# brucefan1983/GPUMD

Measured on AMD Instinct MI355X. Metric: atom-steps/sec, NEP PbTe NVE (nep4 2 Te Pb, examples/nep_train/nep.txt), higher is better.
Workload: dtype f32

## Files before the change

gpumd_amd/csrc/capi_impl.h:

```cpp
#pragma once
#include "../../include/nepmi.h"
#include "engine_impl.h"

#include <exception>
#include <string>

struct nepmi_api;
#if defined(NEPMI_CAPI_DISPATCH)
extern "C" const nepmi_api nepmi_self_api;
#define NEPMI_SELF_API (&nepmi_self_api)
#else
#define NEPMI_SELF_API nullptr
#endif

struct nepmi_model {
  const nepmi_api* api;
  nepmi::NepModel m;
};

struct nepmi_engine {
  const nepmi_api* api;
  nepmi::EngineT<NepmiBackend>* e;
};

// ... 525 lines not shown
    return guarded([&] { eng.set_force_generic(iv != 0); });
  if (n == "tiles")
    eng.set_tile_mode(iv < 0 ? -1 : iv > 2 ? 2 : iv);
  else if (n == "win_lanes")
    eng.set_win_lanes(iv);
  else if (n == "win_max_atoms")
    eng.set_win_max_atoms(iv);
  else if (n == "scatter_guard")
    eng.set_scatter_guard_delayed(value, eng.take_guard_delay());
  else if (n == "scatter_guard_hard")
    eng.set_scatter_guard(-1.0, value);
  else if (n == "scatter_guard_delay")
    eng.set_guard_delay(iv);
  else if (n == "radial_mask")
    eng.set_radial_mask(iv != 0);
  else if (n == "radial_sync")
    eng.set_radial_sync(iv != 0);
  else if (n == "angular_fused")
    eng.set_angular_fused(iv != 0);
  else if (n == "angular_pair_trip")
    eng.set_angular_pair_trip(iv != 0);
  else if (n == "fold_seam")
    eng.set_fold_seam(iv != 0);
  else if (n == "brick_force") {
    if (iv != 0 && !eng.has_brick_force())
      return fail(NEPMI_ERR_ARG, "option 'brick_force': the per-brick force kernel is not part of this build (make BRICK=1)");
    eng.set_brick_force(iv != 0);
  }
  else if (n == "win_static")
    eng.set_win2(iv != 0);
  else if (n == "stepwise_loops")
    eng.set_stepwise_loops(iv != 0);
  else if (n == "mfma")
    eng.set_use_mfma(iv);
  else if (n == "angular_recompute")
    eng.set_angular_recompute(iv);
  else
    return fail(NEPMI_ERR_ARG, "unknown engine option '" + n + "'");
  return NEPMI_OK;
}

}
```

gpumd_amd/csrc/engine.hip:

```cpp
#include <hip/hip_runtime.h>
#include <hiprand/hiprand_kernel.h>

#include <cstring>
#include <stdexcept>
#include <string>

#include "engine_impl.h"
#include "nep_scatter.h"
#include "nep_fused.h"
#ifndef NEPMI_WITH_BRICK
#define NEPMI_WITH_BRICK 0
#endif
#if NEPMI_WITH_BRICK
#include "experimental/nep_brick.h"
#endif

namespace nepmi {

#define NEPMI_HIP_CHECK(expr)                                                                       \
  do {                                                                                              \
    hipError_t err__ = (expr);                                                                      \
    if (err__ != hipSuccess)                                                                        \
      throw std::runtime_error(std::string("HIP error: ") + hipGetErrorString(err__) + " at " +     \
                               __FILE__ + ":" + std::to_string(__LINE__) + " (" #expr ")");         \
// ... 292 lines not shown
  const unsigned per_xcd = gridDim.x >> 3;
  const int64_t wg = (int64_t)(blockIdx.x & 7u) * per_xcd + (blockIdx.x >> 3);
  const int64_t i0 = wg * 128;
  if (i0 >= n)
    return;
  const int tid = (int)threadIdx.x;
  const int64_t i = i0 + (tid >> 1);
  const bool live = i < n;
  const int64_t k = body.b.tperm[live ? i : i0];
  const int t1 = body.b.posq[k].type;
  const int64_t ilast = i0 + 127 < n ? i0 + 127 : n - 1;
  const int t_lo = body.b.posq[body.b.tperm[i0]].type, t_hi = body.b.posq[body.b.tperm[ilast]].type;
  for (int tb = t_lo; tb <= t_hi; tb += kFusedWindowTypes) {
    const int nt = body.m.T - tb < kFusedWindowTypes ? body.m.T - tb : kFusedWindowTypes;
    __syncthreads();
    body.stage_window(nepmi_lds_window, tb, nt, tid, 256);
    __syncthreads();
    if (live && t1 >= tb && t1 < tb + nt)
      body.run_window(k, tid & 1, (lds_cfloat_ptr)nepmi_lds_window, tb);
  }
}
#endif

template <int BLOCK, class Body>
__global__ void __launch_bounds__(BLOCK) __attribute__((amdgpu_waves_per_eu(Body::kMinWavesPerEuPairs)))
nepmi_kernel_lds_pairs_sorted(const Body body, const int64_t n, const int* frozen)
{
  extern __shared__ __attribute__((aligned(16))) float nepmi_lds_pairs_s[];
  __shared__ int hist[64];
  __shared__ unsigned short perm[BLOCK / 2];
  if (frozen && *frozen != 0)
    return;
  const int tid = (int)threadIdx.x;
  body.lds_stage(nepmi_lds_pairs_s, tid, BLOCK);
  if (tid < 64)
    hist[tid] = 0;
  const unsigned per_xcd = gridDim.x >> 3;
  const unsigned tile = (blockIdx.x & 7u) * per_xcd + (blockIdx.x >> 3);
  const int64_t base = (int64_t)tile * (BLOCK / 2);
  const int j = tid >> 1;
  const bool live = base + j < n;
  int key = 0;
  if (live) {
    key = body.sort_key(base + j);
    key = key > 63 ? 63 : key;
    if (tile & 1u)
      key = 63 - key;
  }
  __syncthreads();
  if (live && (tid & 1) == 0)
    atomicAdd(&hist[key], 1);
  __syncthreads();
  if (tid == 0) {
    int run = 0;
    for (int c = 63; c >= 0; --c) {
      const int h = hist[c];
      hist[c] = run;
      run += h;
    }
  }
  __syncthreads();
  if (live && (tid & 1) == 0)
    perm[atomicAdd(&hist[key], 1)] = (unsigned short)j;
  __syncthreads();
  if (live)
    body.template run_parts<2>(base + perm[j], tid & 1, (lds_cfloat_ptr)nepmi_lds_pairs_s);
}

template <class Body>
__global__ void __launch_bounds__(256) nepmi_fused_image(const Body body, float* img)
{
  body.lds_stage(img, (int)threadIdx.x, 256);
}

template <int BLOCK, int P, class Body>
__global__ void __launch_bounds__(BLOCK) nepmi_kernel_lds_parts(const Body body, const int64_t n, const int* frozen)
{
  extern __shared__ __attribute__((aligned(16))) float nepmi_lds_parts[];
  if (frozen && *frozen != 0)
    return;
  const unsigned per_xcd = gridDim.x >> 3;
  const unsigned tile = (blockIdx.x & 7u) * per_xcd + (blockIdx.x >> 3);
  const int64_t i = ((int64_t)tile * BLOCK + threadIdx.x) / P;
  if (i < n)
    body.template run_parts<P>(i, (int)(threadIdx.x % P), (lds_cfloat_ptr)nepmi_lds_parts);
}

template <int BLOCK>
__device__ __forceinline__ int block_exclusive_scan(int v, int* total);
// ... 991 lines not shown
    hipLaunchKernelGGL((nepmi_kernel_lds<BLOCK, Body>), dim3((unsigned)grid), dim3(BLOCK), lds_bytes, stream, body, n, frozen);
    NEPMI_HIP_CHECK(hipGetLastError());
    if (t)
      timer_stop(timing->slot[slot]);
  }

  template <int BLOCK, int P, class Body>
  void launch_lds_parts(int slot, int64_t n, const Body& body)
  {
    if (n <= 0)
      return;
    const int64_t grid = ((P * n + BLOCK - 1) / BLOCK + 7) / 8 * 8;
    const size_t lds_bytes = ((size_t)body.lds_floats() * sizeof(float) + 15) / 16 * 16;
    const bool t = timed(slot);
    if (t)
      timer_start(timing->slot[slot]);
    hipLaunchKernelGGL((nepmi_kernel_lds_parts<BLOCK, P, Body>), dim3((unsigned)grid), dim3(BLOCK), lds_bytes, stream, body, n,
                       frozen);
    NEPMI_HIP_CHECK(hipGetLastError());
    if (t)
      timer_stop(timing->slot[slot]);
  }

  template <int BLOCK, class Body, bool SORTED = false>
  void launch_lds_pairs(int slot, int64_t n, const Body& body)
  {
    if (n <= 0)
      return;
    const int64_t grid = ((2 * n + BLOCK - 1) / BLOCK + 7) / 8 * 8;
    const size_t lds_bytes = ((size_t)body.lds_floats() * sizeof(float) + 15) / 16 * 16;
    void (*kern)(const Body, const int64_t, const int*) = nullptr;
    if constexpr (SORTED)
      kern = &nepmi_kernel_lds_pairs_sorted<BLOCK, Body>;
    else
      kern = &nepmi_kernel_lds_pairs<BLOCK, Body>;
    if (lds_bytes > 60 * 1024)
      NEPMI_HIP_CHECK(hipFuncSetAttribute(reinterpret_cast<const void*>(kern), hipFuncAttributeMaxDynamicSharedMemorySize, (int)lds_bytes));
    const bool t = timed(slot);
    if (t)
      timer_start(timing->slot[slot]);
    hipLaunchKernelGGL(kern, dim3((unsigned)grid), dim3(BLOCK), lds_bytes, stream, body, n, frozen);
    NEPMI_HIP_CHECK(hipGetLastError());
    if (t)
      timer_stop(timing->slot[slot]);
  }

  template <class S>
  size_t fused_image_floats(const ModelD& md) const
  {
    return (size_t)fused_lds_layout<S>(md).total;
  }
  template <class S>
  void launch_angular_fused(int slot, int64_t n, const ModelD& md, const Bufs& b, int export_qfp, float* img, bool build, bool pair_trip)
  {
    AngularFusedBody<S> body{md, b, export_qfp, nullptr};
    if (build) {
      hipLaunchKernelGGL((nepmi_fused_image<AngularFusedBody<S>>), dim3(1), dim3(256), 0, stream, body, img);
      NEPMI_HIP_CHECK(hipGetLastError());
    }
    body.img = img;
#ifndef NEPMI_AFU_BLOCK
#define NEPMI_AFU_BLOCK 256
#endif
#ifndef NEPMI_AFU_SORT
#define NEPMI_AFU_SORT 0
#endif
    if constexpr (FusedShape<S>::NLOC <= kFusedTripMaxChannels) {
      if (pair_trip) {
        launch_lds_pairs<NEPMI_AFU_BLOCK, AngularFusedBody<S, 1>, NEPMI_AFU_SORT != 0>(slot, n, AngularFusedBody<S, 1>{md, b, export_qfp, img});
        return;
      }
    }
    launch_lds_pairs<NEPMI_AFU_BLOCK, AngularFusedBody<S>, NEPMI_AFU_SORT != 0>(slot, n, body);
  }

  template <class S>
  size_t fused_window_lds_bytes(const ModelD& md) const
  {
    return (size_t)fused_lds_layout<S>(md, kFusedWindowTypes).total * sizeof(float);
  }
  static constexpr bool kHasFusedWindow = NEPMI_WITH_FUSED_WINDOW != 0;
  template <class S>
  void launch_angular_fused_window(int slot, int64_t n, const ModelD& md, const Bufs& b, int export_qfp, float* img, bool build)
  {
#if NEPMI_WITH_FUSED_WINDOW
    if (n <= 0)
      return;
    AngularFusedBody<S> body{md, b, export_qfp, nullptr};
    if (build) {
      hipLaunchKernelGGL((nepmi_fused_image<AngularFusedBody<S>>), dim3(1), dim3(256), 0, stream, body, img);
      NEPMI_HIP_CHECK(hipGetLastError());
    }
    body.img = img;
    body.tw = kFusedWindowTypes;
    const int64_t grid = ((n + 127) / 128 + 7) / 8 * 8;
    const size_t lds_bytes = (fused_window_lds_bytes<S>(md) + 15) / 16 * 16;
// ... 438 lines not shown
```

gpumd_amd/csrc/engine_impl.h:

```cpp
#pragma once
#include "nep_bodies.h"
#include "nep_md.h"
#include "nep_model.h"
#include "nep_window.h"
#include "nep_highl.h"
#include "tersoff_bodies.h"

#include <cmath>
#include <cstdio>
#include <cstring>
#include <string>
#include <random>
#include <vector>

#ifndef NEPMI_TERSOFF_SEAM
#define NEPMI_TERSOFF_SEAM 1
#endif
#ifndef NEPMI_WIN2_DEFAULT
#define NEPMI_WIN2_DEFAULT 1
#endif

#define NEPMI_UNPAREN(...) __VA_ARGS__
#if defined(NEPMI_JIT_CORE)
#define NEPMI_SHAPE_DISPATCH(FN, GENERIC, ARGS)                                   \
// ... 995 lines not shown
    const double ras = m.rc_angular_max + kSkin;
    b_.MN_ang = (int)(1.5 * m.MN_angular * ras * ras * ras / (m.rc_angular_max * m.rc_angular_max * m.rc_angular_max)) + 4;
    if (b_.MN_ang > b_.MN_skin)
      b_.MN_ang = b_.MN_skin;
    if (b_.MN_ang > 65000)
      throw EngineError{-3, "angular Verlet list capacity above 65000 slots is not supported"};
    b_.rc_skin_sq = (float)(rcs * rcs);
    b_.rc_askin_sq = (float)(ras * ras);
    b_.cid = dalloc<int>(N);
    b_.kcell = dalloc<int>(N);
    b_.perm = dalloc<int>(N);
    b_.posq = dalloc<PosQ>(N);
    b_.x0s = dalloc<double>(3 * N);
    b_.nn_skin = dalloc<int>(N);
    b_.nl_skin = dalloc<int>((size_t)b_.MN_skin * N);
    b_.code_skin = dalloc<unsigned short>((size_t)b_.MN_skin * N);
    b_.nn_ang = dalloc<int>(N);
    b_.nl_ang = dalloc<int>((size_t)b_.MN_ang * N);
    b_.code_ang = dalloc<unsigned short>((size_t)b_.MN_ang * N);
    b_.rev_ang = dalloc<unsigned short>((size_t)b_.MN_ang * N);
    b_.nn_rad = dalloc<int>(N);
    b_.nn_angstep = dalloc<int>(N);
    b_.nn_angtrue = dalloc<int>(N);
    if (m.kind == 0) {
      b_.rstash = dalloc<F4>((size_t)(b_.MN_ang + b_.MN_skin) * N);
      b_.acomp = dalloc<F4>((size_t)b_.MN_arows * N);
      b_.amap = dalloc<unsigned short>((size_t)b_.MN_ang * N);
      b_.f12 = dalloc<F4>((size_t)b_.MN_arows * N);
      b_.q = dalloc<float>((size_t)m.dim * N);
      b_.fp = dalloc<float>((size_t)m.dim * N);
      b_.sbuf = dalloc<float>((size_t)(m.n_max_angular + 1) * kNumHarm * N);
      b_.shi = m.L_max > 4 ? dalloc<float>((size_t)(m.n_max_angular + 1) * kHighSums * N) : nullptr;
      b_.KRP = ((m.basis_size_radial + 1) + 3) / 4 * 4;
      b_.atab = dalloc<float>((size_t)N * m.num_types * b_.KRP);
      const AnnMfmaShape as = ann_mfma_shape(m.num_types, m.dim, m.num_neurons, b_.KRP);
      b_.ann_img = as.ok ? dalloc<float>(as.img_floats * m.num_types) : nullptr;
      be_.ann_prepare(md_, b_);
      b_.pe_i = dalloc<float>(N);
      b_.MN_rad = m.MN_radial;
      b_.ccode = dalloc<unsigned short>((size_t)b_.MN_rad * N);
      b_.nn_t0 = dalloc<int>(N);
      b_.prec = dalloc<WinRec>(N);
      b_.aidx = dalloc<unsigned short>((size_t)b_.MN_acomp * N);
      b_.amask = dalloc<unsigned>(4 * (size_t)N);
      b_.MN_wchunks = (b_.MN_ang + 3) / 4 + 2 * ((b_.MN_skin + 3) / 4) + 4;
      b_.wcode = dalloc<unsigned short>((size_t)b_.MN_wchunks * 4 * N);
// ... 411 lines not shown
    if constexpr (B::kHasFusedWindow && B::kHasFusedAngular && S::fixed && S::TS == 0) {
      const size_t need = be_.template fused_image_floats<S>(md_);
      if (!fused_img_ || fused_img_floats_ < need) {
        dfree(fused_img_);
        fused_img_ = dalloc<float>(need);
        fused_img_floats_ = need;
        fused_img_stale_ = true;
      }
      be_.template launch_angular_fused_window<S>(kSlotAngular, N_, md_, b_, export_qfp, fused_img_, fused_img_stale_);
      fused_img_stale_ = false;
    }
  }
  template <class S>
  void launch_angular_fused(int export_qfp = 0)
  {
    if constexpr (B::kHasFusedAngular && S::fixed) {
      const size_t need = be_.template fused_image_floats<S>(md_);
      if (!fused_img_ || fused_img_floats_ < need) {
        dfree(fused_img_);
        fused_img_ = dalloc<float>(need);
        fused_img_floats_ = need;
        fused_img_stale_ = true;
      }
      be_.template launch_angular_fused<S>(kSlotAngular, N_, md_, b_, export_qfp, fused_img_, fused_img_stale_, ang_pair_trip_);
      fused_img_stale_ = false;
    }
  }

  template <class S>
  bool brick_force_wanted(const WinStage& ws2) const
  {
    if constexpr (!(B::kHasBrickForce && S::fixed && S::TS == 2)) {
      return false;
    } else {
      if (!brick_force_ || !ang_fused_active() || b_.level || b_.use_rmask || b_.use_csync || !scatter_wanted<S>(ws2))
        return false;
      return be_.template brick_lds_bytes<S>(md_, win_.wmax) <= B::kMaxLdsBytes;
    }
  }
  template <class S>
  void launch_brick_force(const WinStage& ws2, const int* frozen)
  {
    if constexpr (B::kHasBrickForce && S::fixed && S::TS == 2) {
      if (fused_img_stale_ || !fused_img_) {
        launch_angular_fused<S>(0);
      }
      be_.template launch_brick_force<S>(kSlotAngular, kSlotForce, num_bricks_, N_, ws2, md_, halo_, fmap_, fold_rows_, step_outputs_,
// ... 122 lines not shown
    fused_img_stale_ = true;
  }
  double temperature() const { return temperature_; }
  bool temperature_model() const { return model_.temperature_model; }
  int recompute_s() const
  {
    return recompute_mode_ < 0 ? (model_.MN_angular <= 16 ? 1 : 0) : (recompute_mode_ ? 1 : 0);
  }
  void adopt_from(const EngineT& o)
  {
    use_tiles_ = o.use_tiles_;
    tile_mode_ = o.tile_mode_;
    recompute_mode_ = o.recompute_mode_;
    win_lanes_ = o.win_lanes_;
    win_max_atoms_ = o.win_max_atoms_;
    use_win2_ = o.use_win2_;
    external_skin_ = o.external_skin_;
    force_form_ = o.force_form_;
    use_rmask_ = o.use_rmask_;
    use_csync_ = o.use_csync_;
    ang_fused_ = o.ang_fused_;
    ang_pair_trip_ = o.ang_pair_trip_;
    fold_seam_ = o.fold_seam_;
    brick_force_ = o.brick_force_;
    loop_ctx_ = o.loop_ctx_;
    scatter_disabled_ = o.scatter_disabled_;
    b_.scatter_limit = o.b_.scatter_limit;
    b_.fold_guard = o.b_.fold_guard;
    b_.scatter_hard = o.b_.scatter_hard;
    b_.fold_hard = o.b_.fold_hard;
    hard_factor_ = o.hard_factor_;
    hard_asked_ = o.hard_asked_;
    guard_delay_ = o.guard_delay_;
    guard_delayed_ = o.guard_delayed_;
    if (reverse_ghosts_ != o.reverse_ghosts_)
      set_reverse_ghosts(o.reverse_ghosts_);
    unwrapped_ = o.unwrapped_;
    nhc_fresh_ = o.nhc_fresh_;
    bdp_rng_ = o.bdp_rng_;
    bdp_iset_ = o.bdp_iset_;
    bdp_gset_ = o.bdp_gset_;
    lan_seed_ = o.lan_seed_;
    num_compute = o.num_compute;
    num_rebuild = o.num_rebuild;
    num_discarded = o.num_discarded;
    num_range_handovers = o.num_range_handovers;
// ... 335 lines not shown
  }
  bool scatter_enabled() const { return !scatter_disabled_; }
  void clear_range_hard()
  {
    int ov = 0;
    be_.d2h(&ov, b_.flags + kFlagOverflow, sizeof(int));
    if (ov & kOverflowRangeHard) {
      ov &= ~kOverflowRangeHard;
      be_.h2d(b_.flags + kFlagOverflow, &ov, sizeof(int));
    }
  }
  void disable_scatter()
  {
    if (!scatter_disabled_)
      ++num_range_handovers;
    scatter_disabled_ = true;
    be_.memset(b_.flags + kFlagRange, 0, sizeof(int));
  }
  bool last_scatter_form() const { return last_scatter_form_; }
  void set_angular_fused(bool on) { ang_fused_ = on; }
  void set_angular_pair_trip(bool on) { ang_pair_trip_ = on; }
  bool ang_pair_trip_active() const { return ang_pair_trip_ && (model_.n_max_angular + 2) / 2 <= 4; }
  void set_fold_seam(bool on) { fold_seam_ = on; }
  void set_brick_force(bool on) { brick_force_ = on; }
  static constexpr bool has_brick_force() { return B::kHasBrickForce; }
  void set_loop_context(bool on) { loop_ctx_ = on; }
  void set_step_outputs(bool on) { step_outputs_ = on; }
  bool loop_context() const { return loop_ctx_; }
  void exact_virials()
  {
    if (!virial_local_ || model_.kind != 0 || last_small_)
      return;
    be_.frozen = nullptr;
    NEPMI_SHAPE_DISPATCH(exact_virials_shape, 1, ())
  }
  bool virial_local() const { return virial_local_; }

private:
  template <class S>
  void compact_lists_shape()
  {
    const bool padded_rows = b_.use_csync != 0;
    force_kernels_shape<S>(kPhaseRadialOnly, nullptr);
    if (padded_rows)
      angular_kernels<S>();
  }
// ... 71 lines not shown
    } else {
      if (shape_ == 7 || shape_ == 8 || shape_ == 9) {
        s += shape_ == 7 ? "shape=cover(8,12,8,12,6;T)" : (shape_ == 8 ? "shape=cover(12,16,10,12,6;T)" : "shape=cover(8,12,8,12,6;2)");
        if (model_.embedded()) {
          char eb[128];
          std::snprintf(eb, sizeof eb, "<-zero_padded_model(%d,%d,%d,%d,%d)", model_.file_n_max_radial, model_.file_basis_size_radial,
                        model_.file_n_max_angular, model_.file_basis_size_angular, model_.file_num_L);
          s += eb;
        }
      } else {
        s += std::string("shape=") + shapes[shape_ >= 0 && shape_ <= 5 ? shape_ : 0];
      }
    }
    if (last_small_)
      return s + " path=small_box(all image pairs)";
    const int lanes = win_lanes();
    const bool win2 = win2_ok_ && lanes == 1;
    s += tile_ok_ ? (win2 ? " window=lds_static" : " window=lds_scanned") : " window=none(gather kernels)";
    s += " lanes_per_atom=" + std::to_string(tile_ok_ ? lanes : 1);
    if (last_brick_)
      s += " force=one_kernel_per_brick(descriptor+ann+partial_forces+lds_scatter_of_own_halves,lane_pairs)";
    else if (last_ang_fused_)
      s += last_ang_window_ ? " angular=descriptor+ann+partial_forces_in_one_kernel(lane_pairs,sums_in_registers,type_sorted,window_of_4_types)"
                            : (ang_pair_trip_active() ? " angular=descriptor+ann+partial_forces_in_one_kernel(lane_pairs,sums_in_registers,two_record_trips)"
                                              : " angular=descriptor+ann+partial_forces_in_one_kernel(lane_pairs,sums_in_registers)");
    else if (fuse_ann_active())
      s += " ann=fused_with_angular_descriptor(packed_fp32,no_mfma)";
    else if (ann_mode_ != 0 && b_.ann_img && (model_.num_types <= 4 || b_.skip_atab))
      s += model_.num_types > 4 ? " ann=mfma_f32_32x32x2(one_type_per_workgroup)" : " ann=mfma_f32_32x32x2";
    else
      s += " ann=per_atom";
    if (!last_ang_fused_) {
      s += (shape_ != 0 && model_.n_max_angular + 1 >= 7) ? " angular_force=lane_pairs" : " angular_force=one_lane";
      s += recompute_s() ? " angular_sums=recomputed" : " angular_sums=stored";
    }
    s += (last_scatter_form_ && last_mask_form_)   ? " radial_list=inside_bits_over_the_verlet_words"
         : (last_scatter_form_ && last_sync_form_) ? " radial_list=wave_synchronous_words"
                                                   : " radial_list=compacted";
    s += last_scatter_form_ ? (last_fold_seam_ ? " force_assembly=lds_scatter_of_own_halves(fixed_point)+fold_in_integrator_pass"
                                               : " force_assembly=lds_scatter_of_own_halves(fixed_point)+fold") :
         last_rows_form_ ? " force_assembly=table_rows_in_lds"
                         : (last_fpj_form_ ? " force_assembly=neighbour_half_from_fp_rows" : " force_assembly=table_rows_gathered");
    if (num_seam_vetoes_ > 0)
      s += " seam_vetoes=" + std::to_string(num_seam_vetoes_);
    if (tile_ok_)
      s += " bricks=" + std::to_string(num_bricks_) + " window_slots=" + std::to_string(win_.wmax);
    return s;
  }
// ... 32 lines not shown
      be_.end_region(kRegionForce);
      return;
    }
    NEPMI_SHAPE_DISPATCH(force_kernels_shape, 1, (phase, frozen))
  }

  NepModel model_;
  B be_;
  int64_t cap_;
  int64_t N_;
  ModelD md_{};
  Bufs b_;
  BoxD box_;
  WinLayout win_{0, 0};
  bool win2_ok_ = false, use_win2_ = NEPMI_WIN2_DEFAULT != 0;
  bool use_rows_ = true;
  bool last_rows_form_ = false, last_fpj_form_ = false, last_scatter_form_ = false;
  int force_form_ = -1;
  bool loop_ctx_ = false;
  bool virial_local_ = false;
  double hard_factor_ = 4.0;
  bool ang_fused_ = true;
  bool ang_pair_trip_ = !(std::getenv("NEPMI_ANGULAR_PAIR_TRIP") && std::atoi(std::getenv("NEPMI_ANGULAR_PAIR_TRIP")) == 0);
  bool brick_force_ = false;
  bool last_brick_ = false;
  bool brick_pending_ = false;
  float* fused_img_ = nullptr;
  size_t fused_img_floats_ = 0;
  bool fused_img_stale_ = true;
  bool last_ang_fused_ = false;
  bool use_rmask_ = false;
  bool last_mask_form_ = false;
  bool last_ang_window_ = false;
  bool last_sync_form_ = false;
  int guard_delay_ = 0;
  int guard_delay_next_ = 0;
  bool fold_seam_ = !(std::getenv("NEPMI_FOLD_SEAM") && std::atoi(std::getenv("NEPMI_FOLD_SEAM")) == 0);
  bool fold_defer_ = false;
  bool fold_deferred_ = false;
  static constexpr int kSeamBackoffSteps = 256;
  int seam_backoff_ = 0;
  int64_t num_seam_vetoes_ = 0;
  bool last_fold_seam_ = false;
  bool tersoff_defer_ = false;
  bool tersoff_deferred_ = false;
  int64_t calm_steps_ = 0;
// ... 81 lines not shown
```

gpumd_amd/csrc/nep_bodies.h:

```cpp
#pragma once
#include <type_traits>

#include "nep_dev.h"

namespace nepmi {

struct alignas(16) F4 {
  float x, y, z;
  int w;
};

struct alignas(16) U4 {
  unsigned x, y, z, w;
};

struct alignas(16) WinRec {
  int x, y, z;
  int w;
};

struct WinGeom {
  double inv_unit;
  double cell_frac[3];
  int cv[9];
// ... 48 lines not shown
  int gbx, gby, gbz;
  double rc_inv_cell;
  float rc_skin_sq;
  float rc_askin_sq;
  int* cell_count;
  int* cell_fill;
  int* cell_ghost;
  int* brick_live;
  int* brick_flag;
  int* brick_order;
  int* cid;
  int* perm;
  PosQ* posq;
  double* x0s;
  int MN_skin, MN_ang, MN_acomp;
  int MN_arows;
  int* nn_ang;   int* nl_ang;  unsigned short* rev_ang;
  int* nn_skin;  int* nl_skin;
  unsigned short* code_ang;
  unsigned short* code_skin;
  int* nn_rad;   F4* rstash;
  int* nn_angstep; F4* acomp;
  int* nn_angtrue;
  unsigned short* amap;
  F4* f12;
  float* q;
  float* fp;
  float* sbuf;
  float* shi;
  float* atab;
  int KRP;
  float* ann_img;
  float* pe_i;
  float* zbl;
  int* flags;
  const signed char* level;
  signed char* lvl;
  signed char lvl_desc = 1, lvl_force = 2;
  signed char* angf;
  int* tperm;
  int* tpos;
  int* tcount;
  int* sh_ang;
  double* fo;
  int MN_rad;
  unsigned short* ccode;
// ... 1297 lines not shown
      const float d = sqrtf(dot3f(e.x, e.x, e.y, e.y, e.z, e.z));
      const float rc = (rc1 + m.rc_r[t2]) * 0.5f;
      const float rcinv = fast_rcp(rc);
      float fc;
      cutoff_fc(rcinv, d, fc);
      float fn[S::KRM + 1];
      if (S::fixed)
        basis_fn<S::KRM>(rcinv, d, fc, fn);
      else
        basis_fn_rt(KR, rcinv, d, fc, fn);
      const float* c = m.c_rad + (size_t)(t1 * m.T + t2) * (NR + 1) * (KR + 1);
      for (int n = 0; n <= NR; ++n) {
        float g = 0.0f;
        for (int kk = 0; kk <= KR; ++kk)
          g += fn[kk] * c[n * (KR + 1) + kk];
        q[n] += g;
      }
    }
    for (int n = 0; n <= NR; ++n)
      b.q[(int64_t)n * N + b.tpos[k]] = q[n] * m.qscale[n];
  }
};

template <class S, int PARTS, class LP>
NEPMI_HD void angular_s_sums_scalar(const ModelD& m, const Bufs& b, int64_t k, int t1, LP cang, int part, float* s)
{
  constexpr int NLOC = (S::NAM + PARTS) / PARTS;
  const int64_t N = b.N;
  const int NA = S::fixed ? S::NA : m.NA;
  const int KA = S::fixed ? S::KA : m.KA;
  const float rc1 = m.rc_a[t1];
  const int cstride = cang_stride(m);
#pragma unroll
  for (int a = 0; a < NLOC * kNumHarm; ++a)
    s[a] = 0.0f;
  const int na = b.nn_angstep[k];
  const F4* __restrict__ acomp = b.acomp + k;
  F4 e_next;
  if (na > 0)
    e_next = acomp[0];
  for (int a = 0; a < na; ++a) {
    const F4 e = e_next;
    if (a + 1 < na)
      e_next = acomp[(int64_t)(a + 1) * N];
    if (e.w == kNullRecord)
      continue;
// ... 26 lines not shown
        g = fmaf(fn[kk], c[n * (KA + 1) + kk], g);
      }
#pragma unroll
      for (int h = 0; h < kNumHarm; ++h)
        s[i * kNumHarm + h] = fmaf(g, bh[h], s[i * kNumHarm + h]);
    }
  }
}

template <class S, int PARTS, class LP>
NEPMI_HD void angular_s_sums(const ModelD& m, const Bufs& b, int64_t k, int t1, LP cang, int part, float* s)
{
  if constexpr (!S::fixed) {
    angular_s_sums_scalar<S, PARTS>(m, b, k, t1, cang, part, s);
  } else {
    constexpr int NLOC = (S::NAM + PARTS) / PARTS;
    const int64_t N = b.N;
    const float rc1 = m.rc_a[t1];
    const int cstride = cang_stride(m);
    f2 s2[NLOC * kHarmPairs];
#pragma unroll
    for (int a = 0; a < NLOC * kHarmPairs; ++a)
      s2[a] = bc2(0.0f);
    const int na = b.nn_angstep[k];
    const F4* __restrict__ acomp = b.acomp + k;
    F4 e_next;
    if (na > 0)
      e_next = acomp[0];
    for (int a = 0; a < na; ++a) {
      const F4 e = e_next;
      if (a + 1 < na)
        e_next = acomp[(int64_t)(a + 1) * N];
      if (e.w == kNullRecord)
        continue;
      const int t2 = (int)((unsigned)e.w >> kIdxBits);
      const float x = e.x, y = e.y, z = e.z;
      float d, dinv;
      dist_and_inv(dot3f(x, x, y, y, z, z), d, dinv);
      const float rc = m.uniform_rc ? m.rc_a_max : (rc1 + m.rc_a[t2]) * 0.5f;
      const float rcinv = fast_rcp(rc);
      float fc;
      cutoff_fc(rcinv, d, fc);
      float fn[S::KAM + 1];
      basis_fn<S::KAM>(rcinv, d, fc, fn);
      f2 bh[kHarmPairs];
      harmonics_pairs(x * dinv, y * dinv, z * dinv, bh);
      LP c = cang + (t1 * m.T + t2) * cstride;
// ... 15 lines not shown
    const int hp[kNumHarm] = NEPMI_HARM_PAIR_INIT;
#pragma unroll
    for (int i = 0; i < NLOC; ++i)
#pragma unroll
      for (int q = 0; q < kHarmPairs; ++q) {
        s[i * kNumHarm + hp[2 * q]] = s2[i * kHarmPairs + q].x;
        s[i * kNumHarm + hp[2 * q + 1]] = s2[i * kHarmPairs + q].y;
      }
  }
}

template <class S, class LP>
NEPMI_HD void angular_s_sums_trip(const ModelD& m, const Bufs& b, int64_t k, int t1, LP cang, int part, float* s)
{
  static_assert(S::fixed, "compiled shapes only");
  constexpr int NLOC = (S::NA + 2) / 2;
  const int64_t N = b.N;
  const float rc1 = m.rc_a[t1];
  const int cstride = cang_stride(m);
  f2 s2[NLOC * kHarmPairs];
#pragma unroll
  for (int a = 0; a < NLOC * kHarmPairs; ++a)
    s2[a] = bc2(0.0f);
  const int na = b.nn_angstep[k];
  const F4* __restrict__ acomp = b.acomp + k;
  F4 e_next;
  e_next.x = e_next.y = e_next.z = 1.0f;
  e_next.w = kNullRecord;
  if (part < na)
    e_next = acomp[(int64_t)part * N];
  for (int a = 0; a < na; a += 2) {
    const F4 e = e_next;
    e_next.w = kNullRecord;
    if (a + 2 + part < na)
      e_next = acomp[(int64_t)(a + 2 + part) * N];
    const int wA = NEPMI_PAIR_EVEN(e.w), wB = NEPMI_PAIR_ODD(e.w);
    if (wA == kNullRecord && wB == kNullRecord)
      continue;
    const int t2 = e.w != kNullRecord ? (int)((unsigned)e.w >> kIdxBits) : 0;
    const float x = e.x, y = e.y, z = e.z;
    float d, dinv;
    dist_and_inv(dot3f(x, x, y, y, z, z), d, dinv);
    const float rc = m.uniform_rc ? m.rc_a_max : (rc1 + m.rc_a[t2]) * 0.5f;
    const float rcinv = fast_rcp(rc);
    float fc;
    cutoff_fc(rcinv, d, fc);
    float fn[S::KA + 1];
// ... 461 lines not shown
    const int NA = S::fixed ? S::NA : m.NA;
    const int KA = S::fixed ? S::KA : m.KA;
    const float rc1 = m.rc_a[t1];
    const int cstride = cang_stride(m);
    constexpr int NG2 = S::fixed ? NLOC * kHarmPairs : 1;
    f2 G2[NG2];
    if constexpr (S::fixed) {
      const int hp[kNumHarm] = NEPMI_HARM_PAIR_INIT;
#pragma unroll
      for (int i = 0; i < NLOC; ++i)
#pragma unroll
        for (int q = 0; q < kHarmPairs; ++q)
          G2[i * kHarmPairs + q] = mk2(G[i * kNumHarm + hp[2 * q]], G[i * kNumHarm + hp[2 * q + 1]]);
    }

    float zf[3] = {0, 0, 0}, zv[6] = {0, 0, 0, 0, 0, 0}, zpe = 0.0f;
    float pzi = 0.0f;
    int zi = 0;
    if (m.zbl_enabled) {
      zi = m.atomic_number[t1];
      pzi = powf((float)zi, 0.23f);
    }

    const int na = b.nn_angstep[k];
    const F4* __restrict__ acomp = b.acomp + k;
    F4 e_next;
    if (na > 0)
      e_next = acomp[0];
    for (int a = 0; a < na; ++a) {
      const F4 e = e_next;
      if (a + 1 < na)
        e_next = acomp[(int64_t)(a + 1) * N];
      if (e.w == kNullRecord)
        continue;
      const int t2 = (int)((unsigned)e.w >> kIdxBits);
      const float x = e.x, y = e.y, z = e.z;
      float d, dinv;
      dist_and_inv(dot3f(x, x, y, y, z, z), d, dinv);
      const float rc = m.uniform_rc ? m.rc_a_max : (rc1 + m.rc_a[t2]) * 0.5f;
      const float rcinv = fast_rcp(rc);
      float fc, fcp;
      cutoff_fc_fcp(rcinv, d, fc, fcp);
      float fn[S::KAM + 1], fnp[S::KAM + 1];
      if (S::fixed)
        basis_fn_fnp<S::KAM>(rcinv, d, fc, fcp, fn, fnp);
      else
        basis_fn_fnp_rt(KA, rcinv, d, fc, fcp, fn, fnp);
// ... 96 lines not shown
    if (m.zbl_enabled) {
      zi = m.atomic_number[t1];
      pzi = powf((float)zi, 0.23f);
    }
    auto share = [&](const f2* gg, float rx, float ry, float rz, float& w, float& vx, float& vy, float& vz) __attribute__((always_inline)) {
      f2 P2[kHarmPairs], Q2[kHarmPairs];
#pragma unroll
      for (int q = 0; q < kHarmPairs; ++q)
        P2[q] = Q2[q] = bc2(0.0f);
#pragma unroll
      for (int i = 0; i < NLOC; ++i) {
        if (part + 2 * i > S::NA)
          break;
        const f2 g2 = bc2(gg[i].x), gp2 = bc2(gg[i].y);
#pragma unroll
        for (int q = 0; q < kHarmPairs; ++q) {
          P2[q] = vfma(G2[i * kHarmPairs + q], g2, P2[q]);
          Q2[q] = vfma(G2[i * kHarmPairs + q], gp2, Q2[q]);
        }
      }
      harmonics_contract_pairs(rx, ry, rz, P2, Q2, w, vx, vy, vz);
    };

    const int na = b.nn_angstep[k];
    const F4* __restrict__ acomp = b.acomp + k;
    F4 e_next;
    e_next.x = e_next.y = e_next.z = 1.0f;
    e_next.w = kNullRecord;
    if (part < na)
      e_next = acomp[(int64_t)part * N];
    for (int a = 0; a < na; a += 2) {
      const F4 e = e_next;
      e_next.w = kNullRecord;
      if (a + 2 + part < na)
        e_next = acomp[(int64_t)(a + 2 + part) * N];
      const bool own = e.w != kNullRecord, partner = NEPMI_PAIR_XCHG(e.w) != kNullRecord;
      if (!own && !partner)
        continue;
      const int t2 = own ? (int)((unsigned)e.w >> kIdxBits) : 0;
      const float x = e.x, y = e.y, z = e.z;
      float d, dinv;
      dist_and_inv(dot3f(x, x, y, y, z, z), d, dinv);
      const float rc = m.uniform_rc ? m.rc_a_max : (rc1 + m.rc_a[t2]) * 0.5f;
      const float rcinv = fast_rcp(rc);
      float fc, fcp;
      cutoff_fc_fcp(rcinv, d, fc, fcp);
      float fn[S::KA + 1], fnp[S::KA + 1];
// ... 335 lines not shown
```

gpumd_amd/csrc/nep_fused.h:

```cpp
#pragma once
#include "nep_window.h"

namespace nepmi {

template <class S>
struct FusedShape {
  static_assert(S::fixed, "compiled shapes only");
  static constexpr int NRH = (S::NR + 2) / 2;
  static constexpr int NLOC = (S::NA + 2) / 2;
  static constexpr int DPH = (NRH + S::NL * NLOC + 3) / 4 * 4;
  NEPMI_HD static int component(int part, int i)
  {
    if (i < NRH) {
      const int n = 2 * i + part;
      return n <= S::NR ? n : -1;
    }
    const int ii = i - NRH, L = ii / NLOC, c = ii - L * NLOC, n = 2 * c + part;
    if (L >= S::NL || n > S::NA)
      return -1;
    return (S::NR + 1) + L * (S::NA + 1) + n;
  }
};

constexpr int kFusedTripMaxChannels = 4;
// ... 78 lines not shown
    for (int idx = tid; idx < m.T * per_t; idx += nth) {
      const int t = idx / per_t, r = idx - t * per_t;
      const int j = r / (2 * F::DPH), pi = r - j * (2 * F::DPH);
      const int p = pi / F::DPH, i = pi - p * F::DPH;
      const int d = F::component(p, i);
      dst[a.off_w + t * a.wstride + r] = d >= 0 ? m.w0[((size_t)t * m.nneu + j) * m.dim + d] : 0.0f;
    }
    for (int idx = tid; idx < m.T * m.nneu; idx += nth) {
      dst[a.off_b0 + idx] = m.b0[idx];
      dst[a.off_w1 + idx] = m.w1[idx];
    }
    for (int idx = tid; idx < m.T * m.T * (m.NR + 1) * (m.KR + 1); idx += nth)
      dst[a.off_c + idx] = m.c_rad[idx];
    for (int idx = tid; idx < 2 * F::DPH; idx += nth) {
      const int d = F::component(idx / F::DPH, idx % F::DPH);
      dst[a.off_qs + idx] = d >= 0 ? m.qscale[d] : 0.0f;
    }
  }

  NEPMI_HD int sort_key(int64_t k) const
  {
    if (b.lvl[k] < b.lvl_desc)
      return 0;
    return (b.use_csync && b.nn_angtrue) ? b.nn_angtrue[k] : b.nn_angstep[k];
  }
  template <int PARTS, class LP>
  NEPMI_HD void run_parts(int64_t k, int part, LP lds) const
  {
    static_assert(PARTS == 2, "lane pairs");
    run_window(k, part, lds, 0);
  }
  template <class LP>
  NEPMI_HD void run_window(int64_t k, int part, LP lds, int tb) const
  {
    constexpr int NLOC = F::NLOC, DPH = F::DPH;
    if (b.lvl[k] < b.lvl_desc)
      return;
    const int t1 = b.posq[k].type;
    LP cang = lds - tb * m.T * cang_stride(m);
    float s[NLOC * kNumHarm], Fp[DPH], e;
    descriptor_and_ann(k, part, lds, cang, t1, t1 - tb, s, Fp, e);
    if (part == 0)
      b.pe_i[k] = e;
    if (b.fpr) {
#pragma unroll
      for (int i = 0; i < F::NRH; ++i) {
        const int n = 2 * i + part;
// ... 191 lines not shown
```

gpumd_amd/csrc/nep_window.h:

```cpp
#pragma once
#include "nep_bodies.h"

namespace nepmi {

constexpr int kWinThreads = 256;
#ifndef NEPMI_BIGWIN_RADIAL
#define NEPMI_BIGWIN_RADIAL 1024
#endif
#ifndef NEPMI_BIGWIN_SCATTER
#define NEPMI_BIGWIN_SCATTER 768
#endif
constexpr int kWinThreadsBig = NEPMI_BIGWIN_RADIAL;
constexpr int kWinThreadsBigScatter = NEPMI_BIGWIN_SCATTER;
constexpr size_t kBigWindowLds = 80 * 1024;
#ifndef NEPMI_MIDWIN
#define NEPMI_MIDWIN 1
#endif
constexpr int kWinThreadsMid = 512;
constexpr size_t kMidWindowLds = 54 * 1024;
constexpr int kWinCells = 512;
constexpr int kWinMaxAtoms = 6656;

#if defined(__HIP_DEVICE_COMPILE__)
#define NEPMI_LDS(T) __attribute__((address_space(3))) T
// ... 766 lines not shown
  NEPMI_HD bool ctab_on() const { return NEPMI_RW_CTAB && S::TS == 0 && ctab_offset() + 4 * ctab_floats() <= 80 * 1024; }
  NEPMI_HD int lds_bytes() const { return ctab_on() ? ctab_offset() + 4 * ctab_floats() : st.lay.bytes(); }
  NEPMI_HD int64_t map_brick(int64_t w) const { return first < 0 ? w : (int64_t)st.b.brick_order[first + w]; }
  NEPMI_HD bool skip() const { return frozen && *frozen != 0; }
  template <class LC>
  NEPMI_HD void stage(int64_t brick, LC lds, int tid, int nth) const
  {
    if (st.b.brick_live && !st.b.brick_live[brick])
      return;
    st.stage_direct(brick, lds, tid, nth);
    if (ctab_on())
      ctab_stage_padded(m, lds + ctab_offset(), tid, nth, false);
  }
  NEPMI_HD void brick_range(int64_t brick, int64_t& a0, int64_t& a1) const { st.brick_range(brick, a0, a1); }

  template <class LC>
  NEPMI_HD void compute(int64_t brick, int64_t k, LC lds) const
  {
    const Bufs& b = st.b;
    const int64_t N = b.N;
    if (b.lvl[k] < 1) {
      b.nn_rad[k] = 0;
      b.nn_angstep[k] = 0;
      return;
    }
    NEPMI_LDS(const WinRec)* wrec = (NEPMI_LDS(const WinRec)*)(lds + st.lay.off_rec());
    const bool ctab = ctab_on();
    NEPMI_LDS(const float)* ctab_lds = (NEPMI_LDS(const float)*)(lds + ctab_offset());
    const int NR = S::fixed ? S::NR : m.NR;
    const int KR = S::fixed ? S::KR : m.KR;
    const PosQ p1 = b.posq[k];
    const int t1 = p1.type;
    int ox, oy, oz;
    st.place_own(k, ox, oy, oz);
    const float rc1 = m.rc_r[t1], rca1 = m.rc_a[t1];
    const float unit = st.b.wg.unit, unit2 = st.b.wg.unit2, band = st.b.wg.band;
    constexpr int TSM = S::TS > 0 ? S::TS : 1;
    constexpr bool ZIP = S::TS == 2;
    float q[S::NRM + 1];
#pragma unroll
    for (int n = 0; n <= S::NRM; ++n)
      q[n] = 0.0f;

    const int na = b.nn_ang[k];
    const bool owned = b.lvl[k] >= (b.compact_all ? 1 : b.lvl_force);
    const int seg = b.wseg[k];
// ... 140 lines not shown
    const unsigned long long sent64 = 0x0001000100010001ull * (unsigned long long)(unsigned)b.wsent;
    auto sync_emit = [&](SyncFifo& f, U2w* __restrict__& at) __attribute__((always_inline)) {
      const unsigned long long w = f.pop_word(sent64);
      if (f.rows < b.MN_cw) {
        U2w v;
        v.lo = (unsigned)w;
        v.hi = (unsigned)(w >> 32);
        *at = v;
        at += N;
      }
      ++f.rows;
    };
    auto sync_check = [&]() __attribute__((always_inline)) {
      if (SYNC) {
        if (NEPMI_WAVE_ANY(q0.p > 4))
          sync_emit(q0, sync0);
        if (S::TS == 2 && NEPMI_WAVE_ANY(q1.p > 4))
          sync_emit(q1, sync1);
      }
    };
    constexpr bool ASYNC = SYNC != 0 && S::fixed;
    SyncFifo qa;
    qa.init();
    int arows = 0;
    auto ang_emit = [&]() __attribute__((always_inline)) {
      const unsigned slot = qa.pop_one((unsigned)b.wsent);
      if (arows < b.MN_arows) {
        F4 e;
        e.x = e.y = e.z = 0.0f;
        e.w = kNullRecord;
        if (slot != (unsigned)b.wsent) {
          const WinRec r = wrec[slot];
          e.x = (float)(r.x - ox) * unit;
          e.y = (float)(r.y - oy) * unit;
          e.z = (float)(r.z - oz) * unit;
          e.w = r.w;
        }
        acomp[(int64_t)arows * N] = e;
        b.aslot[(int64_t)arows * N + k] = (unsigned short)slot;
      }
      ++arows;
    };
    auto push_front = [&](const Cand& c, const int bit) __attribute__((always_inline)) {
      if (SYNC) {
        if (c.inside) {
          q0.push((unsigned)c.slot);
          ++cnt;
        }
        return;
      }
      if (b.use_rmask) {
        mcur |= c.inside ? (1u << bit) : 0u;
        cnt += c.inside ? 1 : 0;
        return;
// ... 301 lines not shown
        } else if (wide) {
          accumulate_wide(c, 4);
        } else {
#pragma unroll
          for (int u = 0; u < 4; ++u)
            accumulate1(c[u]);
        }
      }
    }

    flush_words();
    if (SYNC) {
      while (NEPMI_WAVE_ANY(q0.p > 0))
        sync_emit(q0, sync0);
      while (S::TS == 2 && NEPMI_WAVE_ANY(q1.p > 0))
        sync_emit(q1, sync1);
    }
    if (ca > b.MN_acomp || (ASYNC && arows > b.MN_arows) || (SYNC ? (q0.rows > b.MN_cw || q1.rows > b.MN_cw) : cnt + cnt1 > b.MN_rad)) {
      NEPMI_ATOMIC_OR(&b.flags[kFlagOverflow], 4);
      ca = ca > b.MN_acomp ? b.MN_acomp : ca;
    }
    if (ASYNC) {
      b.nn_angtrue[k] = ca;
      ca = arows < b.MN_arows ? arows : b.MN_arows;
    }
    b.nn_rad[k] = cnt + cnt1;
    if (SYNC) {
      const int r0 = q0.rows < b.MN_cw ? q0.rows : b.MN_cw, r1 = q1.rows < b.MN_cw ? q1.rows : b.MN_cw;
      b.nn_t0[k] = r0 | (r1 << 8);
    } else {
      b.nn_t0[k] = cnt;
    }
    b.nn_angstep[k] = ca;
    if (S::TS > 0) {
      float Ssum[TSM][S::KRM + 1];
#pragma unroll
      for (int kk = 0; kk <= S::KRM; ++kk) {
        if (ZIP) {
          Ssum[0][kk] = SS[kk].x;
          Ssum[TSM - 1][kk] = SS[kk].y;
        } else {
          Ssum[0][kk] = SS[kk].x + SS[kk].y;
        }
      }
      for (int tu = 0; tu < m.T; ++tu) {
        if (!NEPMI_WAVE_ANY(t1 == tu))
// ... 857 lines not shown
```

gpumd_amd/nep.py:

```python
import ctypes as C

import numpy as np

from . import _capi


def _h9(box):
    h = np.ascontiguousarray(np.asarray(box, dtype=np.float64).reshape(9))
    return h, h.ctypes.data_as(_capi.c_dp)


def _pbc3(pbc):
    p = np.ascontiguousarray(np.asarray(pbc, dtype=np.int32).reshape(3))
    return p, p.ctypes.data_as(_capi.c_ip)


class Model:

    def __init__(self, path, lib=None):
        from . import load_library
        self.lib = lib if lib is not None else load_library()
        self.path = path
        self.handle = self.lib.nepmi_model_load(path.encode())
        if not self.handle:
# ... 252 lines not shown

    def set_radial_sync(self, on=True):
        self.set_option("radial_sync", 1 if on else 0)

    def set_scatter_guard(self, ev_per_angstrom=64.0, hard_factor=0.0):
        self.set_option("scatter_guard", float(ev_per_angstrom))
        self.set_option("scatter_guard_hard", float(hard_factor))

    def set_virial_mode(self, mode=0):
        self._ck(self.lib.nepmi_engine_set_virial_mode(self.handle, int(mode)))

    def set_brick_force(self, on=True):
        self.set_option("brick_force", 1 if on else 0)

    def set_angular_fused(self, on=True):
        self.set_option("angular_fused", 1 if on else 0)

    def set_angular_pair_trip(self, on=True):
        self.set_option("angular_pair_trip", 1 if on else 0)

    def set_fold_seam(self, on=True):
        self.set_option("fold_seam", 1 if on else 0)

    def describe(self):
        import ctypes as C
        buf = C.create_string_buffer(512)
        n = self.lib.nepmi_engine_describe(self.handle, buf, 512)
        if n < 0:
            self._ck(n)
        return buf.value.decode()

    def set_stepwise_loops(self, on=True):
        self.set_option("stepwise_loops", int(bool(on)))

    def set_win_static(self, on=True):
        self.set_option("win_static", int(bool(on)))

    def set_mfma(self, on=True):
        self.set_option("mfma", int(on))

    def set_temperature(self, temperature):
        self._ck(self.lib.nepmi_engine_set_temperature(self.handle, float(temperature)))

    def set_angular_recompute(self, mode=-1):
        self.set_option("angular_recompute", int(mode))

# ... 3 lines not shown
```

Before: 955.1 million.

## Add count-sorted single-wave pool kernel for fused angular and trim walk rows

Replaces the unused sorted-pairs angular kernel with a 64-lane pool kernel. It sorts 128 atoms by neighbor count using a wave-scan histogram and then loops over 32-atom slices, so lane pairs carry balanced work. The pool path is opt-in through the angular_pool option or the NEPMI_ANGULAR_POOL env var, and with pool=1 it also needs at least 500k atoms and a check that it uses no more scratch. Separately, the window builder now records the last non-null angular row (nn_anglast), and the angular walkers use it in the csync path, so trailing null rows are no longer iterated. That second change runs by default, and it also changes the fused kernel's sort_key from nn_angtrue to nn_anglast.

Result: no change. 957.0 million, median of 6 (+0.2%).

```diff
diff --git a/gpumd_amd/csrc/capi_impl.h b/gpumd_amd/csrc/capi_impl.h
--- a/gpumd_amd/csrc/capi_impl.h
+++ b/gpumd_amd/csrc/capi_impl.h
@@ -571,6 +571,8 @@
     eng.set_angular_pair_trip(iv != 0);
   else if (n == "fold_seam")
     eng.set_fold_seam(iv != 0);
+  else if (n == "angular_pool")
+    eng.set_angular_pool(iv);
   else if (n == "brick_force") {
     if (iv != 0 && !eng.has_brick_force())
       return fail(NEPMI_ERR_ARG, "option 'brick_force': the per-brick force kernel is not part of this build (make BRICK=1)");
diff --git a/gpumd_amd/csrc/engine.hip b/gpumd_amd/csrc/engine.hip
--- a/gpumd_amd/csrc/engine.hip
+++ b/gpumd_amd/csrc/engine.hip
@@ -338,49 +338,72 @@
 }
 #endif
 
-template <int BLOCK, class Body>
-__global__ void __launch_bounds__(BLOCK) __attribute__((amdgpu_waves_per_eu(Body::kMinWavesPerEuPairs)))
-nepmi_kernel_lds_pairs_sorted(const Body body, const int64_t n, const int* frozen)
-{
-  extern __shared__ __attribute__((aligned(16))) float nepmi_lds_pairs_s[];
+#ifndef NEPMI_AFU_BLOCK
+#define NEPMI_AFU_BLOCK 256
+#endif
+#ifndef NEPMI_AFU_POOL
+#define NEPMI_AFU_POOL 128
+#endif
+constexpr int kPoolSortBytes = 64 * sizeof(int);
+template <int POOL, class Body>
+__global__ void __launch_bounds__(64) __attribute__((amdgpu_waves_per_eu(Body::kMinWavesPerEuPairs)))
+nepmi_kernel_lds_pairs_pool(const Body body, const int64_t n, const int* frozen)
+{
+  static_assert(POOL % 64 == 0 && POOL <= 1024, "whole wavefronts of keys");
+  extern __shared__ __attribute__((aligned(16))) float nepmi_lds_pool[];
   __shared__ int hist[64];
-  __shared__ unsigned short perm[BLOCK / 2];
+  __shared__ unsigned short perm[POOL];
   if (frozen && *frozen != 0)
     return;
-  const int tid = (int)threadIdx.x;
-  body.lds_stage(nepmi_lds_pairs_s, tid, BLOCK);
-  if (tid < 64)
-    hist[tid] = 0;
   const unsigned per_xcd = gridDim.x >> 3;
   const unsigned tile = (blockIdx.x & 7u) * per_xcd + (blockIdx.x >> 3);
-  const int64_t base = (int64_t)tile * (BLOCK / 2);
-  const int j = tid >> 1;
-  const bool live = base + j < n;
-  int key = 0;
-  if (live) {
-    key = body.sort_key(base + j);
-    key = key > 63 ? 63 : key;
-    if (tile & 1u)
-      key = 63 - key;
-  }
-  __syncthreads();
-  if (live && (tid & 1) == 0)
-    atomicAdd(&hist[key], 1);
-  __syncthreads();
-  if (tid == 0) {
-    int run = 0;
-    for (int c = 63; c >= 0; --c) {
-      const int h = hist[c];
-      hist[c] = run;
-      run += h;
-    }
-  }
-  __syncthreads();
-  if (live && (tid & 1) == 0)
-    perm[atomicAdd(&hist[key], 1)] = (unsigned short)j;
-  __syncthreads();
-  if (live)
-    body.template run_parts<2>(base + perm[j], tid & 1, (lds_cfloat_ptr)nepmi_lds_pairs_s);
+  const int64_t base = (int64_t)tile * POOL;
+  if (base >= n)
+    return;
+  const int lane = (int)threadIdx.x;
+  const int live = n - base < POOL ? (int)(n - base) : POOL;
+  body.lds_stage(nepmi_lds_pool, lane, 64);
+  hist[lane] = 0;
+  int key[POOL / 64];
+#pragma unroll
+  for (int u = 0; u < POOL / 64; ++u) {
+    const int j = lane + 64 * u;
+    key[u] = 0;
+    if (j < live) {
+      const int c = body.sort_key(base + j);
+      key[u] = c > 63 ? 63 : c;
+    }
+  }
+  __syncthreads();
+#pragma unroll
+  for (int u = 0; u < POOL / 64; ++u)
+    if (lane + 64 * u < live)
+      atomicAdd(&hist[key[u]], 1);
+  __syncthreads();
+  {
+    const int h = hist[63 - lane];
+    int run = h;
+#pragma unroll
+    for (int d = 1; d < 64; d <<= 1) {
+      const int up = __shfl_up(run, d, 64);
+      run += lane >= d ? up : 0;
+    }
+    hist[63 - lane] = run - h;
+  }
+  __syncthreads();
+#pragma unroll
+  for (int u = 0; u < POOL / 64; ++u)
+    if (lane + 64 * u < live)
+      perm[atomicAdd(&hist[key[u]], 1)] = (unsigned short)(lane + 64 * u);
+  __syncthreads();
+#pragma nounroll
+  for (int s = 0; s < POOL / 32; ++s) {
+    int ln;
+    asm volatile("v_mbcnt_lo_u32_b32 %0, -1, 0\n\tv_mbcnt_hi_u32_b32 %0, -1, %0" : "=v"(ln));
+    const int j = 32 * s + (ln >> 1);
+    if (j < live)
+      body.per_slice().template run_parts<2>(base + perm[j], ln & 1, (lds_cfloat_ptr)nepmi_lds_pool);
+  }
 }
 
 template <class Body>
@@ -1418,18 +1441,14 @@
       timer_stop(timing->slot[slot]);
   }
 
-  template <int BLOCK, class Body, bool SORTED = false>
+  template <int BLOCK, class Body>
   void launch_lds_pairs(int slot, int64_t n, const Body& body)
   {
     if (n <= 0)
       return;
     const int64_t grid = ((2 * n + BLOCK - 1) / BLOCK + 7) / 8 * 8;
     const size_t lds_bytes = ((size_t)body.lds_floats() * sizeof(float) + 15) / 16 * 16;
-    void (*kern)(const Body, const int64_t, const int*) = nullptr;
-    if constexpr (SORTED)
-      kern = &nepmi_kernel_lds_pairs_sorted<BLOCK, Body>;
-    else
-      kern = &nepmi_kernel_lds_pairs<BLOCK, Body>;
+    void (*kern)(const Body, const int64_t, const int*) = &nepmi_kernel_lds_pairs<BLOCK, Body>;
     if (lds_bytes > 60 * 1024)
       NEPMI_HIP_CHECK(hipFuncSetAttribute(reinterpret_cast<const void*>(kern), hipFuncAttributeMaxDynamicSharedMemorySize, (int)lds_bytes));
     const bool t = timed(slot);
@@ -1441,13 +1460,49 @@
       timer_stop(timing->slot[slot]);
   }
 
+  static constexpr int kAngularPool = NEPMI_AFU_POOL;
+  static constexpr int64_t kAngularPoolMinAtoms = 500000;
+  template <class Body>
+  static bool pool_lds_fits(const Body& body)
+  {
+    const size_t bytes = ((size_t)body.lds_floats() * sizeof(float) + 15) / 16 * 16 + kPoolSortBytes + kAngularPool * sizeof(unsigned short);
+    return 8 * ((bytes + 1279) / 1280 * 1280) <= 160 * 1024;
+  }
+  template <class Body>
+  bool pool_without_more_scratch()
+  {
+    static int cached = -1;
+    if (cached < 0) {
+      hipFuncAttributes pool{}, plain{};
+      NEPMI_HIP_CHECK(hipFuncGetAttributes(&pool, reinterpret_cast<const void*>(&nepmi_kernel_lds_pairs_pool<kAngularPool, Body>)));
+      NEPMI_HIP_CHECK(hipFuncGetAttributes(&plain, reinterpret_cast<const void*>(&nepmi_kernel_lds_pairs<NEPMI_AFU_BLOCK, Body>)));
+      cached = pool.localSizeBytes <= plain.localSizeBytes ? 1 : 0;
+    }
+    return cached != 0;
+  }
+  template <class Body>
+  void launch_lds_pairs_pool(int slot, int64_t n, const Body& body)
+  {
+    if (n <= 0)
+      return;
+    const int64_t grid = ((n + kAngularPool - 1) / kAngularPool + 7) / 8 * 8;
+    const size_t lds_bytes = ((size_t)body.lds_floats() * sizeof(float) + 15) / 16 * 16;
+    const bool t = timed(slot);
+    if (t)
+      timer_start(timing->slot[slot]);
+    hipLaunchKernelGGL((nepmi_kernel_lds_pairs_pool<kAngularPool, Body>), dim3((unsigned)grid), dim3(64), lds_bytes, stream, body, n, frozen);
+    NEPMI_HIP_CHECK(hipGetLastError());
+    if (t)
+      timer_stop(timing->slot[slot]);
+  }
+
   template <class S>
   size_t fused_image_floats(const ModelD& md) const
   {
     return (size_t)fused_lds_layout<S>(md).total;
   }
   template <class S>
-  void launch_angular_fused(int slot, int64_t n, const ModelD& md, const Bufs& b, int export_qfp, float* img, bool build, bool pair_trip)
+  int launch_angular_fused(int slot, int64_t n, const ModelD& md, const Bufs& b, int export_qfp, float* img, bool build, bool pair_trip, int pool)
   {
     AngularFusedBody<S> body{md, b, export_qfp, nullptr};
     if (build) {
@@ -1455,19 +1510,24 @@
       NEPMI_HIP_CHECK(hipGetLastError());
     }
     body.img = img;
-#ifndef NEPMI_AFU_BLOCK
-#define NEPMI_AFU_BLOCK 256
-#endif
-#ifndef NEPMI_AFU_SORT
-#define NEPMI_AFU_SORT 0
-#endif
+    bool pooled = pool != 0 && !b.level && pool_lds_fits(body) && (pool >= 2 || n >= kAngularPoolMinAtoms);
     if constexpr (FusedShape<S>::NLOC <= kFusedTripMaxChannels) {
       if (pair_trip) {
-        launch_lds_pairs<NEPMI_AFU_BLOCK, AngularFusedBody<S, 1>, NEPMI_AFU_SORT != 0>(slot, n, AngularFusedBody<S, 1>{md, b, export_qfp, img});
-        return;
+        const AngularFusedBody<S, 1> trips{md, b, export_qfp, img};
+        pooled = pooled && pool_without_more_scratch<AngularFusedBody<S, 1>>();
+        if (pooled)
+          launch_lds_pairs_pool(slot, n, trips);
+        else
+          launch_lds_pairs<NEPMI_AFU_BLOCK>(slot, n, trips);
+        return pooled ? kAngularPool : 0;
       }
     }
-    launch_lds_pairs<NEPMI_AFU_BLOCK, AngularFusedBody<S>, NEPMI_AFU_SORT != 0>(slot, n, body);
+    pooled = pooled && pool_without_more_scratch<AngularFusedBody<S>>();
+    if (pooled)
+      launch_lds_pairs_pool(slot, n, body);
+    else
+      launch_lds_pairs<NEPMI_AFU_BLOCK>(slot, n, body);
+    return pooled ? kAngularPool : 0;
   }
 
   template <class S>
diff --git a/gpumd_amd/csrc/engine_impl.h b/gpumd_amd/csrc/engine_impl.h
--- a/gpumd_amd/csrc/engine_impl.h
+++ b/gpumd_amd/csrc/engine_impl.h
@@ -1041,6 +1041,7 @@
     b_.nn_rad = dalloc<int>(N);
     b_.nn_angstep = dalloc<int>(N);
     b_.nn_angtrue = dalloc<int>(N);
+    b_.nn_anglast = dalloc<int>(N);
     if (m.kind == 0) {
       b_.rstash = dalloc<F4>((size_t)(b_.MN_ang + b_.MN_skin) * N);
       b_.acomp = dalloc<F4>((size_t)b_.MN_arows * N);
@@ -1498,7 +1499,7 @@
         fused_img_floats_ = need;
         fused_img_stale_ = true;
       }
-      be_.template launch_angular_fused<S>(kSlotAngular, N_, md_, b_, export_qfp, fused_img_, fused_img_stale_, ang_pair_trip_);
+      last_ang_pool_ = be_.template launch_angular_fused<S>(kSlotAngular, N_, md_, b_, export_qfp, fused_img_, fused_img_stale_, ang_pair_trip_, ang_pool_);
       fused_img_stale_ = false;
     }
   }
@@ -1667,6 +1668,7 @@
     ang_fused_ = o.ang_fused_;
     ang_pair_trip_ = o.ang_pair_trip_;
     fold_seam_ = o.fold_seam_;
+    ang_pool_ = o.ang_pool_;
     brick_force_ = o.brick_force_;
     loop_ctx_ = o.loop_ctx_;
     scatter_disabled_ = o.scatter_disabled_;
@@ -2048,6 +2050,7 @@
   void set_angular_pair_trip(bool on) { ang_pair_trip_ = on; }
   bool ang_pair_trip_active() const { return ang_pair_trip_ && (model_.n_max_angular + 2) / 2 <= 4; }
   void set_fold_seam(bool on) { fold_seam_ = on; }
+  void set_angular_pool(int v) { ang_pool_ = v < 0 ? 0 : (v > 2 ? 2 : v); }
   void set_brick_force(bool on) { brick_force_ = on; }
   static constexpr bool has_brick_force() { return B::kHasBrickForce; }
   void set_loop_context(bool on) { loop_ctx_ = on; }
@@ -2165,8 +2168,9 @@
       s += " force=one_kernel_per_brick(descriptor+ann+partial_forces+lds_scatter_of_own_halves,lane_pairs)";
     else if (last_ang_fused_)
       s += last_ang_window_ ? " angular=descriptor+ann+partial_forces_in_one_kernel(lane_pairs,sums_in_registers,type_sorted,window_of_4_types)"
-                            : (ang_pair_trip_active() ? " angular=descriptor+ann+partial_forces_in_one_kernel(lane_pairs,sums_in_registers,two_record_trips)"
-                                              : " angular=descriptor+ann+partial_forces_in_one_kernel(lane_pairs,sums_in_registers)");
+                            : (ang_pair_trip_active() ? " angular=descriptor+ann+partial_forces_in_one_kernel(lane_pairs,sums_in_registers,two_record_trips"
+                                                      : " angular=descriptor+ann+partial_forces_in_one_kernel(lane_pairs,sums_in_registers") +
+                                  (last_ang_pool_ > 0 ? ",count_sorted_pools=" + std::to_string(last_ang_pool_) + ")" : std::string(")"));
     else if (fuse_ann_active())
       s += " ann=fused_with_angular_descriptor(packed_fp32,no_mfma)";
     else if (ann_mode_ != 0 && b_.ann_img && (model_.num_types <= 4 || b_.skip_atab))
@@ -2245,6 +2249,8 @@
   double hard_factor_ = 4.0;
   bool ang_fused_ = true;
   bool ang_pair_trip_ = !(std::getenv("NEPMI_ANGULAR_PAIR_TRIP") && std::atoi(std::getenv("NEPMI_ANGULAR_PAIR_TRIP")) == 0);
+  int ang_pool_ = std::getenv("NEPMI_ANGULAR_POOL") ? std::max(0, std::min(2, std::atoi(std::getenv("NEPMI_ANGULAR_POOL")))) : 0;
+  int last_ang_pool_ = 0;
   bool brick_force_ = false;
   bool last_brick_ = false;
   bool brick_pending_ = false;
diff --git a/gpumd_amd/csrc/nep_bodies.h b/gpumd_amd/csrc/nep_bodies.h
--- a/gpumd_amd/csrc/nep_bodies.h
+++ b/gpumd_amd/csrc/nep_bodies.h
@@ -94,6 +94,7 @@
   int* nn_rad;   F4* rstash;
   int* nn_angstep; F4* acomp;
   int* nn_angtrue;
+  int* nn_anglast;
   unsigned short* amap;
   F4* f12;
   float* q;
@@ -1437,6 +1438,12 @@
   }
 };
 
+NEPMI_HD int ang_walk_rows(const Bufs& b, int64_t k)
+{
+  const int* __restrict__ rows = (b.use_csync && b.nn_anglast) ? b.nn_anglast : b.nn_angstep;
+  return rows[k];
+}
+
 template <class S, int PARTS, class LP>
 NEPMI_HD void angular_s_sums_scalar(const ModelD& m, const Bufs& b, int64_t k, int t1, LP cang, int part, float* s)
 {
@@ -1509,7 +1516,7 @@
 #pragma unroll
     for (int a = 0; a < NLOC * kHarmPairs; ++a)
       s2[a] = bc2(0.0f);
-    const int na = b.nn_angstep[k];
+    const int na = ang_walk_rows(b, k);
     const F4* __restrict__ acomp = b.acomp + k;
     F4 e_next;
     if (na > 0)
@@ -1571,7 +1578,7 @@
 #pragma unroll
   for (int a = 0; a < NLOC * kHarmPairs; ++a)
     s2[a] = bc2(0.0f);
-  const int na = b.nn_angstep[k];
+  const int na = ang_walk_rows(b, k);
   const F4* __restrict__ acomp = b.acomp + k;
   F4 e_next;
   e_next.x = e_next.y = e_next.z = 1.0f;
@@ -2079,7 +2086,7 @@
       pzi = powf((float)zi, 0.23f);
     }
 
-    const int na = b.nn_angstep[k];
+    const int na = ang_walk_rows(b, k);
     const F4* __restrict__ acomp = b.acomp + k;
     F4 e_next;
     if (na > 0)
@@ -2222,7 +2229,7 @@
       harmonics_contract_pairs(rx, ry, rz, P2, Q2, w, vx, vy, vz);
     };
 
-    const int na = b.nn_angstep[k];
+    const int na = ang_walk_rows(b, k);
     const F4* __restrict__ acomp = b.acomp + k;
     F4 e_next;
     e_next.x = e_next.y = e_next.z = 1.0f;
diff --git a/gpumd_amd/csrc/nep_fused.h b/gpumd_amd/csrc/nep_fused.h
--- a/gpumd_amd/csrc/nep_fused.h
+++ b/gpumd_amd/csrc/nep_fused.h
@@ -124,7 +124,15 @@
   {
     if (b.lvl[k] < b.lvl_desc)
       return 0;
-    return (b.use_csync && b.nn_angtrue) ? b.nn_angtrue[k] : b.nn_angstep[k];
+    return ang_walk_rows(b, k);
+  }
+  NEPMI_HD AngularFusedBody per_slice() const
+  {
+    AngularFusedBody c = *this;
+#if defined(__HIP_DEVICE_COMPILE__)
+    asm volatile("" : "+s"(c.m.zbl_rc_outer));
+#endif
+    return c;
   }
   template <int PARTS, class LP>
   NEPMI_HD void run_parts(int64_t k, int part, LP lds) const
diff --git a/gpumd_amd/csrc/nep_window.h b/gpumd_amd/csrc/nep_window.h
--- a/gpumd_amd/csrc/nep_window.h
+++ b/gpumd_amd/csrc/nep_window.h
@@ -812,6 +812,8 @@
     if (b.lvl[k] < 1) {
       b.nn_rad[k] = 0;
       b.nn_angstep[k] = 0;
+      if (SYNC != 0 && S::fixed)
+        b.nn_anglast[k] = 0;
       return;
     }
     NEPMI_LDS(const WinRec)* wrec = (NEPMI_LDS(const WinRec)*)(lds + st.lay.off_rec());
@@ -998,7 +1000,7 @@
     constexpr bool ASYNC = SYNC != 0 && S::fixed;
     SyncFifo qa;
     qa.init();
-    int arows = 0;
+    int arows = 0, alast = 0;
     auto ang_emit = [&]() __attribute__((always_inline)) {
       const unsigned slot = qa.pop_one((unsigned)b.wsent);
       if (arows < b.MN_arows) {
@@ -1006,6 +1008,7 @@
         e.x = e.y = e.z = 0.0f;
         e.w = kNullRecord;
         if (slot != (unsigned)b.wsent) {
+          alast = arows + 1;
           const WinRec r = wrec[slot];
           e.x = (float)(r.x - ox) * unit;
           e.y = (float)(r.y - oy) * unit;
@@ -1353,6 +1356,7 @@
     }
     if (ASYNC) {
       b.nn_angtrue[k] = ca;
+      b.nn_anglast[k] = alast;
       ca = arows < b.MN_arows ? arows : b.MN_arows;
     }
     b.nn_rad[k] = cnt + cnt1;
diff --git a/gpumd_amd/nep.py b/gpumd_amd/nep.py
--- a/gpumd_amd/nep.py
+++ b/gpumd_amd/nep.py
@@ -298,6 +298,9 @@
     def set_fold_seam(self, on=True):
         self.set_option("fold_seam", 1 if on else 0)
 
+    def set_angular_pool(self, mode=1):
+        self.set_option("angular_pool", int(mode))
+
     def describe(self):
         import ctypes as C
         buf = C.create_string_buffer(512)
```
